# austin-hoover/ment-flow

Measured on NVIDIA B200. Metric: particles/sec/GPU for flow sample+log_prob+project+KDE (6D, 100 proj), higher is better.
Workload: dtype f32

## Files before the change

include/mentflow_b200.h:

```cpp
#ifndef MENTFLOW_B200_H
#define MENTFLOW_B200_H

#include <stdint.h>

#ifdef __cplusplus
extern "C" {
#endif

#define MFB_ABI_VERSION 2

#define MFB_E_BADARG (-1)
#define MFB_E_UNSUPPORTED (-2)
#define MFB_E_WORKSPACE (-3)

#define MFB_FLAG_NO_TENSOR_CORES 1

int mfb_abi_version(void);
const char* mfb_error_string(int code);
int mfb_sm_count(void);

#define MFB_GEOM_STRIDE 8

int64_t mfb_kde1d_workspace_bytes(int64_t n, int d, int k, int b);
int mfb_project_kde1d_fwd(const float* x, int64_t n, int d, const float* proj, const float* geom,
// ... 133 lines not shown
                          int nb_meas2, int meas_axis2, int n_int_axes, const int32_t* int_shape_host,
                          const float* int_first_host, const float* int_step_host, const float* minv,
                          const float* proj, const float* coords, const float* tables, int k, int b,
                          const float* proj2, const float* cx2, const float* cy2, const float* tables2, int k2,
                          int bx, int by, float prior_neg_half_inv_s2, float prior_log_norm, float* pred,
                          void* stream);
int64_t mfb_cdf_workspace_bytes(int64_t g);
int mfb_cdf_build(const float* rho, int64_t g, double pad, double* cdf, void* workspace,
                  int64_t workspace_bytes, void* stream);
int mfb_cdf_sample(const double* cdf, int64_t g, const void* workspace, int d,
                   const int32_t* shape_host, const float* first_edge_host, const float* cell_host,
                   int jitter, uint64_t seed, uint64_t offset, int64_t size, float* out, void* stream);
int mfb_gs_update(float* table, const float* meas, const float* pred, int n, float lr, float thresh,
                  void* stream);

int64_t mfb_randn_offset_increment(int64_t numel);
int mfb_randn_philox(float* out, int64_t numel, uint64_t seed, uint64_t offset, void* stream);
int mfb_randn_philox_state(float* out, int64_t numel, uint64_t* state, int advance, void* stream);

int mfb_selftest_umma(const float* a, const float* b, int n, float* d, int* err, void* stream);
int mfb_selftest_umma_ts(const float* a, const float* b, int n, float* d, int* err, void* stream);
int mfb_selftest_umma_sw32(const float* a, const float* b, int n, int mode, int kstep, float* d, int* err,
                           void* stream);

#ifdef __cplusplus
}
#endif
#endif
```

mentflow_b200/_lib.py:

```python
import ctypes
import os
from ctypes import c_char_p, c_double, c_float, c_int, c_int64, c_uint64, c_void_p

PKG_DIR = os.path.dirname(os.path.abspath(__file__))
LIB_PATH = os.environ.get("MENTFLOW_B200_LIB") or os.path.join(PKG_DIR, "libmentflow_b200.so")

P = c_void_p

SIGNATURES = {
    "mfb_abi_version": (c_int, []),
    "mfb_error_string": (c_char_p, [c_int]),
    "mfb_sm_count": (c_int, []),
    "mfb_kde1d_workspace_bytes": (c_int64, [c_int64, c_int, c_int, c_int]),
    "mfb_project_kde1d_fwd": (c_int, [P, c_int64, c_int, P, P, c_int, c_int, c_float, P, P, c_int64, P]),
    "mfb_kde1d_normalize": (c_int, [P, c_double, P, c_int, c_int, P, P]),
    "mfb_kde1d_normalize_bwd": (c_int, [P, c_double, P, c_int, c_int, P, P, P]),
    "mfb_project_kde1d_loss_fwd": (c_int, [P, c_int64, c_int, P, P, c_int, c_int, c_float, c_double, P, c_float, P, P, P,
                                           P, c_int64, P]),
    "mfb_kde1d_finish": (c_int, [P, c_double, P, c_int, c_int, P, c_float, P, P, P]),
    "mfb_kde1d_p2p_block_floats": (c_int64, [c_int, c_int, c_int]),
    "mfb_kde1d_finish_p2p": (c_int, [P, c_int, c_int, P, P, P, c_int, c_double, P, c_int, c_int, P, c_float, P, P, P, P, P]),
    "mfb_project_kde1d_loss_fwd_p2p": (c_int, [P, c_int64, c_int, P, P, c_int, c_int, c_float, c_double, P, c_float, P,
                                               c_int, c_int, P, P, c_int, P, P, P, P, P, c_int64, P]),
    "mfb_kde1d_finish_bwd": (c_int, [P, c_double, P, c_int, c_int, P, c_float, P, P, P, P]),
# ... 23 lines not shown
                                  c_int64, c_int, P]),
    "mfb_nsf_layer_bwd_img": (c_int, [P, P, P, c_int64, c_int, c_int, c_int, c_int, P, P, P, c_int, P, P, P, c_int, P,
                                      c_int64, c_int, P]),
    "mfb_ment_prob": (c_int, [P, c_int64, c_int, P, P, P, c_int, c_int, c_float, c_float, P, P]),
    "mfb_ment_prob_grid": (c_int, [c_int, P, P, P, P, P, P, c_int, c_int, c_float, c_float, P, P]),
    "mfb_ment_integrate": (c_int, [c_int, P, c_int, c_int, c_int, P, P, P, P, P, P, P, c_int, c_int, c_float,
                                   c_float, P, P]),
    "mfb_ment_prob_nd": (c_int, [P, c_int64, c_int, P, P, P, c_int, c_int, P, P, P, P, c_int, c_int, c_int, c_float,
                                 c_float, P, P]),
    "mfb_ment_prob_grid_nd": (c_int, [c_int, P, P, P, P, P, P, c_int, c_int, P, P, P, P, c_int, c_int, c_int, c_float,
                                      c_float, P, P]),
    "mfb_ment_integrate_nd": (c_int, [c_int, P, c_int, c_int, P, c_int, c_int, c_int, P, P, P, P, P, P, P, c_int, c_int,
                                      P, P, P, P, c_int, c_int, c_int, c_float, c_float, P, P]),
    "mfb_randn_offset_increment": (c_int64, [c_int64]),
    "mfb_randn_philox": (c_int, [P, c_int64, c_uint64, c_uint64, P]),
    "mfb_randn_philox_state": (c_int, [P, c_int64, P, c_int, P]),
    "mfb_cdf_workspace_bytes": (c_int64, [c_int64]),
    "mfb_cdf_build": (c_int, [P, c_int64, c_double, P, P, c_int64, P]),
    "mfb_cdf_sample": (c_int, [P, c_int64, P, c_int, P, P, P, c_int, c_uint64, c_uint64, c_int64, P, P]),
    "mfb_gs_update": (c_int, [P, P, P, c_int, c_float, c_float, P]),
    "mfb_selftest_umma": (c_int, [P, P, c_int, P, P, P]),
    "mfb_selftest_umma_ts": (c_int, [P, P, c_int, P, P, P]),
    "mfb_selftest_umma_sw32": (c_int, [P, P, c_int, c_int, c_int, P, P, P]),
    "mfb_nsf_pack_params": (c_int, [P, P, P, P, P, P, P, P, P, c_int, c_int, c_int, c_int, c_int, P, P, P]),
    "mfb_nsf_unpack_grads": (c_int, [P, P, P, P, c_int, c_int, c_int, c_int, c_int, P, P, P, P, P, P, P]),
    "mfb_moments_workspace_bytes": (c_int64, [c_int64, c_int]),
    "mfb_moments": (c_int, [P, P, c_int64, c_int, c_int, P, P, c_int64, P]),
    "mfb_f64_split": (c_int, [P, c_int, P, P]),
    "mfb_f64_join": (c_int, [P, c_int, P, P]),
    "mfb_mc_entropy": (c_int, [P, c_double, c_double, c_double, P, P]),
    "mfb_loss_tail": (c_int, [P, c_int, P, c_float, P, P]),
}

_lib = None


class LibraryMissing(RuntimeError):
    pass


def load():
    global _lib
    if _lib is not None:
        return _lib
    if not os.path.exists(LIB_PATH):
        raise LibraryMissing(
# ... 19 lines not shown
```

mentflow_b200/csrc/nsf_spline_regs.cuh:

```cuda
#pragma once
#include <math.h>

#include "nsf_common.cuh"

#define MFB_HD __host__ __device__ __forceinline__

namespace mfb {
namespace tc {

constexpr int kCT = 24;
constexpr int kConstRows = 7;
constexpr int kConstFloats = kConstRows * kCT + kPP;

MFB_HD float sp_exp2(float x) {
#ifdef __CUDA_ARCH__
  float y;
  asm("ex2.approx.ftz.f32 %0, %1;" : "=f"(y) : "f"(x));
  return y;
#else
  return exp2f(x);
#endif
}
MFB_HD float sp_rcp(float x) {
#ifdef __CUDA_ARCH__
// ... 64 lines not shown
  const float d2 = fmaf(fabsf(t2), c, 1.0f), d3 = fmaf(fabsf(t3), c, 1.0f);
  float p01, p23, x0, x1, x2, x3;
  mul2(d0, d2, d1, d3, p01, p23);
  const float r = sp_rcp(p01 * p23);
  const float r01 = r * p23, r23 = r * p01;
  mul2(t0, t1, r01 * d1, r01 * d0, x0, x1);
  mul2(t2, t3, r23 * d3, r23 * d2, x2, x3);
  e0 = sp_exp2(x0);
  e1 = sp_exp2(x1);
  e2 = sp_exp2(x2);
  e3 = sp_exp2(x3);
}

MFB_HD void two_sum(float a, float b, float& s, float& err) {
  s = sp_add(a, b);
  const float bb = sp_add(s, -a);
  err = sp_add(sp_add(a, -sp_add(s, -bb)), sp_add(b, -bb));
}

#ifndef MFB_SPLINE_COMP
#define MFB_SPLINE_COMP 1
#endif

template <int NB>
MFB_HD float rq_spline_regs(const float (&a)[64], float v, float& jac) {
  static_assert(NB % 4 == 0 && NB >= 8, "bins are searched in groups of four");
  constexpr int G = NB / 4;
  constexpr float cW = kClipW / kLog2e, cD = kClipD / kLog2e;
  float e[NB], pre[G + 1], plo[G + 1];
#pragma unroll
  for (int j = 0; j < NB; j += 4) {
    clip_exp2_quad(a[j], a[j + 1], a[j + 2], a[j + 3], cW, e[j], e[j + 1], e[j + 2], e[j + 3]);
  }
  pre[0] = 0.f;
  plo[0] = 0.f;
#pragma unroll
  for (int g = 0; g < G; ++g) {
    float s01, s23;
    add2(e[4 * g], e[4 * g + 2], e[4 * g + 1], e[4 * g + 3], s01, s23);
    const float gs = s01 + s23;
    if (MFB_SPLINE_COMP >= 1 && g > 0) {
      float err;
      two_sum(pre[g], gs, pre[g + 1], err);
      plo[g + 1] = plo[g] + err;
    } else {
      pre[g + 1] = pre[g] + gs;
      plo[g + 1] = 0.f;
    }
  }
  const float sum = pre[G], half = 0.5f * sum;
  const float u = v * (0.5f / kBound);
  const float target = fmaf(u, sum, half);
  bool pg[G - 1];
#pragma unroll
  for (int g = 0; g < G - 1; ++g) pg[g] = pre[g + 1] < target;
  float q0 = e[0], q1 = e[1], q2 = e[2], q3 = e[3], xg = 0.f, xgl = 0.f;
#pragma unroll
  for (int g = 1; g < G; ++g) {
    q0 = pg[g - 1] ? e[4 * g] : q0;
    q1 = pg[g - 1] ? e[4 * g + 1] : q1;
    q2 = pg[g - 1] ? e[4 * g + 2] : q2;
    q3 = pg[g - 1] ? e[4 * g + 3] : q3;
    xg = pg[g - 1] ? pre[g] : xg;
    if (MFB_SPLINE_COMP >= 1) xgl = pg[g - 1] ? plo[g] : xgl;
  }
  float cen = half - xg;
  if (MFB_SPLINE_COMP >= 1) cen += fmaf(0.5f, plo[G], -xgl);
  const float rem = fmaf(u, sum, cen);
  const float i1 = q0 + q1, i2 = i1 + q2;
  const bool r0 = q0 < rem, r1 = i1 < rem, r2 = i2 < rem;
  const float numer = rem - (r2 ? i2 : (r1 ? i1 : (r0 ? q0 : 0.f)));
  const float ek = r2 ? q3 : (r1 ? q2 : (r0 ? q1 : q0));
  float run = 0.f, runl = 0.f, yg = 0.f, ygl = 0.f, h0s = 0.f, h1s = 0.f, h2s = 0.f, h3s = 0.f;
#pragma unroll
  for (int g = 0; g < G; ++g) {
    float h0, h1, h2, h3;
    clip_exp2_quad(a[NB + 4 * g], a[NB + 4 * g + 1], a[NB + 4 * g + 2], a[NB + 4 * g + 3], cW, h0, h1, h2, h3);
    const bool take = g == 0 ? true : pg[g > 0 ? g - 1 : 0];
    h0s = take ? h0 : h0s;
    h1s = take ? h1 : h1s;
    h2s = take ? h2 : h2s;
    h3s = take ? h3 : h3s;
    yg = take ? run : yg;
    float s01, s23;
    add2(h0, h2, h1, h3, s01, s23);
    const float gs = s01 + s23;
    if (MFB_SPLINE_COMP >= 2 && g > 0) {
      ygl = take ? runl : ygl;
      float err;
      two_sum(run, gs, run, err);
      runl += err;
    } else {
      run += gs;
    }
  }
  const float sumh = run;
  const float j1h = h0s + h1s, j2h = j1h + h2s;
  float ycen = (yg - 0.5f * sumh) + (r2 ? j2h : (r1 ? j1h : (r0 ? h0s : 0.f)));
  if (MFB_SPLINE_COMP >= 2) ycen += fmaf(-0.5f, runl, ygl);
  const float hk = r2 ? h3s : (r1 ? h2s : (r0 ? h1s : h0s));
  float um = 0.f, u0 = 0.f, u1 = 0.f, u2 = 0.f, u3 = 0.f, prev = 0.f;
#pragma unroll
  for (int g = 0; g < G; ++g) {
    const float t0 = a[2 * NB + 4 * g], t1 = a[2 * NB + 4 * g + 1], t2 = a[2 * NB + 4 * g + 2];
    const float t3 = (4 * g + 3 < NB - 1) ? a[2 * NB + 4 * g + 3] : 0.f;
    const bool take = g == 0 ? true : pg[g > 0 ? g - 1 : 0];
    um = take ? prev : um;
    u0 = take ? t0 : u0;
    u1 = take ? t1 : u1;
    u2 = take ? t2 : u2;
    u3 = take ? t3 : u3;
    prev = t3;
  }
  const float tl = r2 ? u2 : (r1 ? u1 : (r0 ? u0 : um));
  const float tr = r2 ? u3 : (r1 ? u2 : (r0 ? u1 : u0));
  float d0, d1;
  clip_exp2_pair(tl, tr, cD, d0, d1);
  const float r_e = rcp_nr(ek), r_sh = rcp_nr(sumh);
  float t = numer * r_e;
  t = fminf(fmaxf(t, 0.0f), 1.0f);
  const float hn = hk * r_sh;
  const float s = hn * sum * r_e;
  const float omt = 1.0f - t, tomt = t * omt;
  const float den = fmaf(d0 + d1 - 2.0f * s, tomt, s);
  const float r_den = rcp_nr(den);
  const float y0 = 2.0f * kBound * (ycen * r_sh);
  const float y = fmaf(2.0f * kBound * hn * (s * t * t + d0 * tomt), r_den, y0);
  const float j1 = s * s * (2.0f * s * tomt + d0 * omt * omt + d1 * t * t) * r_den * r_den;
  const bool inside = (v > -kBound) && (v <= kBound);
  jac *= inside ? j1 : 1.0f;
  return inside ? y : v;
}

MFB_HD void clip_exp2_quad_bwd(float& t0, float& t1, float& t2, float& t3, float c, float& e0,
                                                   float& e1, float& e2, float& e3) {
  const float d0 = fmaf(fabsf(t0), c, 1.0f), d1 = fmaf(fabsf(t1), c, 1.0f);
  const float d2 = fmaf(fabsf(t2), c, 1.0f), d3 = fmaf(fabsf(t3), c, 1.0f);
  const float p01 = d0 * d1, p23 = d2 * d3;
  const float r = sp_rcp(p01 * p23);
  const float r01 = r * p23, r23 = r * p01;
  const float i0 = r01 * d1, i1 = r01 * d0, i2 = r23 * d3, i3 = r23 * d2;
  e0 = sp_exp2(t0 * i0);
  e1 = sp_exp2(t1 * i1);
  e2 = sp_exp2(t2 * i2);
  e3 = sp_exp2(t3 * i3);
  t0 = i0; t1 = i1; t2 = i2; t3 = i3;
}

struct KnotGrad {
  float left, right;
  int bin;
};
template <int NB>
MFB_HD float rq_spline_regs_bwd(float (&a)[64], float v, float gy, float gl, KnotGrad* kg = nullptr) {
// ... 242 lines not shown
```

mentflow_b200/csrc/nsf_tc.cu:

```cuda
#include "nsf_spline_regs.cuh"
#include "nsf_tc_common.cuh"

namespace mfb {
namespace tc {


struct Meta {
  int slot_feature[kMaxDim];
  int slot_ksteps[kMaxDim];
  int hid_n0[4];
  int const_feature;
  int nslots;
  int perm[kH];
};

struct BwdIO {
  const float* gy;
  const float* glogq;
  float* acts;
  float* gphi;
  uint32_t* masks;
  float* gvd;
  float* gmax;
  int* gmaxes;
// ... 194 lines not shown
  asm("cvt.rz.relu.f16x2.f32 %0, %1, %2;" : "=r"(hi) : "f"(x1), "f"(x0));
  const __half2 h = *reinterpret_cast<const __half2*>(&hi);
  const float2 hf = __half22float2(h);
  float r0, r1;
  add2(x0, x1, -hf.x, -hf.y, r0, r1);
  asm("cvt.rn.relu.f16x2.f32 %0, %1, %2;" : "=r"(lo) : "f"(r1), "f"(r0));
}

__device__ __forceinline__ void store_hidden(const float (&acc)[64], unsigned char* a_hi, unsigned char* a_lo, int row) {
#pragma unroll
  for (int c = 0; c < 8; ++c) {
    uint32_t hi[4], lo[4];
#pragma unroll
    for (int e = 0; e < 4; ++e) split_relu_pair(acc[8 * c + 2 * e], acc[8 * c + 2 * e + 1], hi[e], lo[e]);
    const uint32_t off = umma::sw128_offset(row, c);
    *reinterpret_cast<uint4*>(a_hi + off) = make_uint4(hi[0], hi[1], hi[2], hi[3]);
    *reinterpret_cast<uint4*>(a_lo + off) = make_uint4(lo[0], lo[1], lo[2], lo[3]);
  }
}

#ifndef MFB_TC_TS
#define MFB_TC_TS 1
#endif
__device__ __forceinline__ void store_hidden_ts(const float (&acc)[64], uint32_t tmem_a_hi, unsigned char* a_lo, int row) {
#pragma unroll
  for (int c2 = 0; c2 < 4; ++c2) {
    uint32_t hi[8];
#pragma unroll
    for (int h = 0; h < 2; ++h) {
      const int c = 2 * c2 + h;
      uint32_t lo[4];
#pragma unroll
      for (int e = 0; e < 4; ++e) split_relu_pair(acc[8 * c + 2 * e], acc[8 * c + 2 * e + 1], hi[4 * h + e], lo[e]);
      *reinterpret_cast<uint4*>(a_lo + umma::sw128_offset(row, c)) = make_uint4(lo[0], lo[1], lo[2], lo[3]);
    }
    umma::tmem_st8(tmem_a_hi + 8 * c2, hi);
  }
  umma::tmem_wait_st();
}

__device__ __forceinline__ void mirror_rows(const unsigned char* a_hi, unsigned char* g_img, int warp_in_wg) {
  __syncwarp();
  if ((threadIdx.x & 31) == 0) {
    const uint32_t off = (uint32_t)warp_in_wg * 4096u;
    asm volatile("cp.async.bulk.global.shared::cta.bulk_group [%0], [%1], 4096;" ::"l"(g_img + off), "r"(smem_u32(a_hi + off)) : "memory");
    asm volatile("cp.async.bulk.global.shared::cta.bulk_group [%0], [%1], 4096;" ::"l"(g_img + kABytes / 2 + off),
                 "r"(smem_u32(a_hi + kABytes / 2 + off))
                 : "memory");
    asm volatile("cp.async.bulk.commit_group;" ::: "memory");
  }
}
__device__ __forceinline__ void mirror_wait() {
  if ((threadIdx.x & 31) == 0) asm volatile("cp.async.bulk.wait_group.read 0;" ::: "memory");
  __syncwarp();
}

__device__ __forceinline__ void mma_slot(uint32_t tmem_d, uint64_t a_hi, uint64_t a_lo, uint64_t b_hi, uint64_t b_lo,
                                         int nk, uint32_t idesc) {
  for (int ks = 0; ks < nk; ++ks) mma_cross(tmem_d, a_hi, a_lo, b_hi, b_lo, ks, idesc, ks > 0);
  for (int ks = 0; ks < nk; ++ks) mma_main(tmem_d, a_hi, b_hi, ks, idesc);
}
// ... 189 lines not shown
    umma::fence_after_sync();
    TRACE(2);
  };
  auto start_tile = [&](const float* vv, uint64_t* landed, uint32_t parity) {
    mbar_wait_bounded(landed, parity);
    if constexpr (kBwd) mirror_wait();
    __align__(16) __half row[16];
#pragma unroll
    for (int e = 0; e < 16; ++e) row[e] = __float2half_rn(0.f);
#pragma unroll
    for (int i = 0; i < D; ++i) umma::split_f16(vv[i], row[i], row[D + i]);
    row[2 * D] = __float2half_rn(1.0f);
    row[2 * D + 1] = __float2half_rn(1.0f);
    *reinterpret_cast<uint4*>(a_hi + umma::sw128_offset(t, 0)) = reinterpret_cast<const uint4*>(row)[0];
    *reinterpret_cast<uint4*>(a_hi + umma::sw128_offset(t, 1)) = reinterpret_cast<const uint4*>(row)[1];
    fence_proxy_async();
    request_arrive(req_chain);
    TRACE(3);
  };
  int64_t next_p = 0;
  bool next_valid = false;
  auto hidden_step = [&](int l) {
    wait_buf(kHB);
    float acc[64];
    tmem_ld64(col0 + (uint32_t)(kHB * 64) + lane_sel, acc);
    if constexpr (kBwd) mirror_wait();
    if constexpr (kTS) store_hidden_ts(acc, ta_hi + lane_sel, a_lo, t);
    else store_hidden(acc, a_hi, a_lo, t);
    fence_proxy_async();
    umma::fence_before_sync();
    request_arrive(req_chain);
    if constexpr (kBwd) {
      mirror_rows(a_hi, reinterpret_cast<unsigned char*>(bio.acts) + ((size_t)(next_p >> 7) * L + l) * kABytes, t >> 5);
      if (next_valid) {
        uint32_t m0 = 0, m1 = 0;
#pragma unroll
        for (int c = 0; c < 64; ++c) {
          if (c < 32) m0 |= (acc[c] > 0.f ? 1u : 0u) << c;
          else m1 |= (acc[c] > 0.f ? 1u : 0u) << (c - 32);
        }
        uint32_t* mk = bio.masks + ((size_t)(next_p >> 7) * (L * 2) + l * 2) * 128 + t;
        mk[0] = m0;
        mk[128] = m1;
      }
    }
    TRACE(4 + l);
  };

  float* stage0 = stage_all + ((size_t)(wg * 2) * 128 + t) * D;
  float* stage1 = stage0 + 128 * D;
  uint64_t* sbar = sbars + 2 * wg;
// ... 10 lines not shown
    if (bulk) tma_load_1d(dst, src, bulk, &sbar[buf]);
  };

  int64_t tile = first_tile_of(wg);
  bool cur = false;
  bool has_next = tile < ntiles;
  float* sc = stage0;
  float* sn = stage1;
  int nbuf = 1;
  uint32_t sph0 = 0, sph1 = 0;
  float jac_carry = 1.0f, ss_carry = 0.f;
  if (t == 0) prefetch(tile, nbuf);
  tile -= tstride;
  while (cur || has_next) {
    const int64_t p = tile * 128 + t;
    const bool valid = cur && p < n;
    if (cur) has_next = tile + tstride < ntiles;
    next_p = (tile + tstride) * 128 + t;
    next_valid = has_next && next_p < n;
    float jac = jac_carry;
    float ss = ss_carry;
    float lq_in = 0.f;
    if (!kBwd && cur && valid && logq_out && !first_layer) lq_in = logq_in[p];
    float gyr[D], glq = 0.f, amax = 0.f;
    if constexpr (kBwd) {
#pragma unroll
      for (int i = 0; i < D; ++i) gyr[i] = valid ? bio.gy[p * D + i] : 0.f;
      glq = (valid && bio.glogq) ? bio.glogq[p] : 0.f;
    }
    auto feature_bwd = [&](float (&acc)[64], int f) {
      const float vf = sc[f];
      float gyf = gyr[0];
#pragma unroll
      for (int i = 1; i < D; ++i) gyf = (f == i) ? gyr[i] : gyf;
      KnotGrad kg;
      float gvf = rq_spline_regs_bwd<NB>(acc, vf, gyf, -glq, &kg);
      if (first_layer) gvf -= glq * vf;
      sc[f] = gvf;
      if (valid) {
        float* gp = bio.gphi + ((size_t)tile * (D * kGRows) + f * kGRows) * 128 + t;
#pragma unroll
        for (int j = 0; j < 2 * NB; ++j) {
          gp[j * 128] = acc[j];
          amax = fmaxf(amax, fabsf(acc[j]));
        }
        gp[(2 * NB) * 128] = kg.left;
        gp[(2 * NB + 1) * 128] = kg.right;
        gp[(2 * NB + 2) * 128] = (float)kg.bin;
        amax = fmaxf(amax, fmaxf(fabsf(kg.left), fabsf(kg.right)));
      }
    };
#pragma unroll 1
    for (int s = kBwd ? -1 : 0; s < S; ++s) {
      const int b = s & 1;
      float acc[64];
      if (kBwd && s < 0) {
        if (cur) {
          const float4* cb = reinterpret_cast<const float4*>(ctab + kConstRows * kCT);
#pragma unroll
          for (int i = 0; i < 16; ++i) {
            const float4 q4 = cb[i];
            acc[4 * i] = q4.x; acc[4 * i + 1] = q4.y; acc[4 * i + 2] = q4.z; acc[4 * i + 3] = q4.w;
          }
        }
      } else if (cur) {
        if (!(S >= 2 && s == S - 1)) wait_buf(b);
        tmem_ld64(col0 + (uint32_t)(b * 64) + lane_sel, acc);
        umma::fence_before_sync();
        if (s + 2 < S) request_arrive(req_chain + 1 + b);
        if (s == 0 && t == 0 && has_next) prefetch(tile + tstride, nbuf);
        TRACE(10 + s);
      }
      if (s == kFork) {
        if (cur && S >= 2) wait_buf((S - 1) & 1);
        if (has_next) {
          if (nbuf == 0) {
            start_tile(sn, &sbar[0], sph0);
            sph0 ^= 1;
          } else {
            start_tile(sn, &sbar[1], sph1);
            sph1 ^= 1;
          }
        }
      }
      if (cur) {
        const int f = (kBwd && s < 0) ? meta.const_feature : meta.slot_feature[s < 0 ? 0 : s];
        if constexpr (kBwd) {
          feature_bwd(acc, f);
        } else {
          const float vf = sc[f];
          ss = fmaf(vf, vf, ss);
          sc[f] = rq_spline_regs<NB>(acc, vf, jac);
        }
        TRACE(20 + s);
      }
      if (has_next) {
        if (s == kFork) hidden_step(0);
        if (S >= 2 && s == S - 1) hidden_step(1);
      }
    }
    if (S == 1 && has_next) hidden_step(1);
    if constexpr (kBwd) {
      if (valid) {
#pragma unroll
        for (int i = 0; i < D; ++i) bio.gvd[p * D + i] = sc[i];
        bio.gmax[p] = amax;
      }
      if (cur) {
        float wm = valid ? amax : 0.f;
#pragma unroll
        for (int o = 16; o > 0; o >>= 1) wm = fmaxf(wm, __shfl_xor_sync(0xffffffffu, wm, o));
        if ((t & 31) == 0) atomicMax(bio.gmaxes, __float_as_int(wm));
      }
      if (has_next) hidden_step(2);
    } else {
      if (valid) {
#pragma unroll
// ... 471 lines not shown
```

mentflow_b200/csrc/nsf_tc_common.cuh:

```cuda
#pragma once
#include "nsf_common.cuh"
#include "umma.cuh"

namespace mfb {
namespace tc {

constexpr int kWG = 3;
constexpr int kThreads = (kWG + 1) * 128;
constexpr int kRegsCompute = 160, kRegsIssuer = 32;
constexpr int kTileBytes = 8192;
constexpr int kABytes = 32768;
constexpr int kGRowsOf(int nb) { return 2 * nb + 4; }
constexpr int kGRows = kGRowsOf(20);

#ifndef MFB_TC_DEAL_BY_WG
#define MFB_TC_DEAL_BY_WG 1
#endif
__device__ __forceinline__ int64_t first_tile_of(int wg) {
#if MFB_TC_DEAL_BY_WG
  return (int64_t)wg * gridDim.x + blockIdx.x;
#else
  return (int64_t)blockIdx.x * kWG + wg;
#endif
}
// ... 49 lines not shown
__device__ __forceinline__ void tmem_ld64(uint32_t taddr, float (&v)[64]) {
  uint32_t r[64];
  asm volatile(
      "tcgen05.ld.sync.aligned.32x32b.x64.b32 "
      "{%0, %1, %2, %3, %4, %5, %6, %7, %8, %9, %10, %11, %12, %13, %14, %15, "
      "%16, %17, %18, %19, %20, %21, %22, %23, %24, %25, %26, %27, %28, %29, %30, %31, "
      "%32, %33, %34, %35, %36, %37, %38, %39, %40, %41, %42, %43, %44, %45, %46, %47, "
      "%48, %49, %50, %51, %52, %53, %54, %55, %56, %57, %58, %59, %60, %61, %62, %63}, [%64];"
      : "=r"(r[0]), "=r"(r[1]), "=r"(r[2]), "=r"(r[3]), "=r"(r[4]), "=r"(r[5]), "=r"(r[6]), "=r"(r[7]), "=r"(r[8]),
        "=r"(r[9]), "=r"(r[10]), "=r"(r[11]), "=r"(r[12]), "=r"(r[13]), "=r"(r[14]), "=r"(r[15]), "=r"(r[16]),
        "=r"(r[17]), "=r"(r[18]), "=r"(r[19]), "=r"(r[20]), "=r"(r[21]), "=r"(r[22]), "=r"(r[23]), "=r"(r[24]),
        "=r"(r[25]), "=r"(r[26]), "=r"(r[27]), "=r"(r[28]), "=r"(r[29]), "=r"(r[30]), "=r"(r[31]), "=r"(r[32]),
        "=r"(r[33]), "=r"(r[34]), "=r"(r[35]), "=r"(r[36]), "=r"(r[37]), "=r"(r[38]), "=r"(r[39]), "=r"(r[40]),
        "=r"(r[41]), "=r"(r[42]), "=r"(r[43]), "=r"(r[44]), "=r"(r[45]), "=r"(r[46]), "=r"(r[47]), "=r"(r[48]),
        "=r"(r[49]), "=r"(r[50]), "=r"(r[51]), "=r"(r[52]), "=r"(r[53]), "=r"(r[54]), "=r"(r[55]), "=r"(r[56]),
        "=r"(r[57]), "=r"(r[58]), "=r"(r[59]), "=r"(r[60]), "=r"(r[61]), "=r"(r[62]), "=r"(r[63])
      : "r"(taddr)
      : "memory");
  asm volatile("tcgen05.wait::ld.sync.aligned;" ::: "memory");
#pragma unroll
  for (int i = 0; i < 64; ++i) v[i] = __uint_as_float(r[i]);
}

__device__ __forceinline__ void mma_cross(uint32_t tmem_d, uint64_t a_hi, uint64_t a_lo, uint64_t b_hi, uint64_t b_lo,
                                          int kstep, uint32_t idesc, uint32_t accumulate) {
  umma::mma_f16_ss(tmem_d, umma::desc_advance_k(a_hi, kstep), umma::desc_advance_k(b_lo, kstep), idesc, accumulate);
  umma::mma_f16_ss(tmem_d, umma::desc_advance_k(a_lo, kstep), umma::desc_advance_k(b_hi, kstep), idesc, 1);
}
__device__ __forceinline__ void mma_main(uint32_t tmem_d, uint64_t a_hi, uint64_t b_hi, int kstep, uint32_t idesc) {
  umma::mma_f16_ss(tmem_d, umma::desc_advance_k(a_hi, kstep), umma::desc_advance_k(b_hi, kstep), idesc, 1);
}
__device__ __forceinline__ void store_split8(unsigned char* hi_tile, unsigned char* lo_tile, int row, int chunk,
                                             const float (&x)[8]) {
  __align__(16) __half hi[8], lo[8];
#pragma unroll
  for (int e = 0; e < 8; ++e) umma::split_f16(x[e], hi[e], lo[e]);
  const uint32_t off = umma::sw128_offset(row, chunk);
  *reinterpret_cast<uint4*>(hi_tile + off) = *reinterpret_cast<const uint4*>(hi);
  *reinterpret_cast<uint4*>(lo_tile + off) = *reinterpret_cast<const uint4*>(lo);
}
static void hidden_classes(int d, int* cls, int* perm) {
  for (int h = 0; h < kH; ++h) cls[h] = 1 + h % (d - 1);
  int p = 0;
  for (int c = 1; c <= d - 1; ++c)
    for (int h = 0; h < kH; ++h)
      if (cls[h] == c) perm[p++] = h;
// ... 5 lines not shown
```

mentflow_b200/csrc/umma.cuh:

```cuda
#pragma once
#include <cuda_fp16.h>

#include "common.cuh"

namespace mfb {
namespace umma {

__device__ __forceinline__ uint32_t sw128_offset(int r, int c) {
  return (uint32_t)((r >> 3) * 1024 + (r & 7) * 128 + ((c ^ (r & 7)) << 4));
}

__device__ __forceinline__ uint64_t make_desc_sw128(uint32_t smem_addr) {
  uint64_t d = (uint64_t)((smem_addr & 0x3FFFFu) >> 4);
  d |= (uint64_t)1 << 16;
  d |= (uint64_t)(1024 >> 4) << 32;
  d |= (uint64_t)1 << 46;
  d |= (uint64_t)2 << 61;
  return d;
}
__device__ __forceinline__ uint64_t desc_advance_k(uint64_t desc, int kstep) { return desc + (uint64_t)(kstep * 2); }

__device__ __forceinline__ uint32_t sw32_offset(int r, int c) {
  return (uint32_t)(r * 32 + ((c ^ ((r >> 2) & 1)) << 4));
}
// ... 50 lines not shown
}
__device__ __forceinline__ void tmem_st4(uint32_t taddr, const uint32_t (&r)[4]) {
  asm volatile("tcgen05.st.sync.aligned.32x32b.x4.b32 [%0], {%1, %2, %3, %4};" ::"r"(taddr), "r"(r[0]), "r"(r[1]), "r"(r[2]),
               "r"(r[3])
               : "memory");
}
__device__ __forceinline__ void tmem_wait_st() { asm volatile("tcgen05.wait::st.sync.aligned;" ::: "memory"); }
__device__ __forceinline__ void commit(uint64_t* bar) {
  asm volatile("tcgen05.commit.cta_group::1.mbarrier::arrive::one.shared::cluster.b64 [%0];" ::"r"(smem_u32(bar))
               : "memory");
}
__device__ __forceinline__ void fence_before_sync() { asm volatile("tcgen05.fence::before_thread_sync;" ::: "memory"); }
__device__ __forceinline__ void fence_after_sync() { asm volatile("tcgen05.fence::after_thread_sync;" ::: "memory"); }

__device__ __forceinline__ void tmem_alloc(uint32_t* dst, uint32_t cols) {
  asm volatile("tcgen05.alloc.cta_group::1.sync.aligned.shared::cta.b32 [%0], %1;" ::"r"(smem_u32(dst)), "r"(cols)
               : "memory");
  asm volatile("tcgen05.relinquish_alloc_permit.cta_group::1.sync.aligned;" ::: "memory");
}
__device__ __forceinline__ void tmem_dealloc(uint32_t addr, uint32_t cols) {
  asm volatile("tcgen05.dealloc.cta_group::1.sync.aligned.b32 %0, %1;" ::"r"(addr), "r"(cols) : "memory");
}

__device__ __forceinline__ void tmem_ld32(uint32_t taddr, float (&v)[32]) {
  uint32_t r[32];
  asm volatile(
      "tcgen05.ld.sync.aligned.32x32b.x32.b32 "
      "{%0, %1, %2, %3, %4, %5, %6, %7, %8, %9, %10, %11, %12, %13, %14, %15, "
      "%16, %17, %18, %19, %20, %21, %22, %23, %24, %25, %26, %27, %28, %29, %30, %31}, [%32];"
      : "=r"(r[0]), "=r"(r[1]), "=r"(r[2]), "=r"(r[3]), "=r"(r[4]), "=r"(r[5]), "=r"(r[6]), "=r"(r[7]), "=r"(r[8]),
        "=r"(r[9]), "=r"(r[10]), "=r"(r[11]), "=r"(r[12]), "=r"(r[13]), "=r"(r[14]), "=r"(r[15]), "=r"(r[16]),
        "=r"(r[17]), "=r"(r[18]), "=r"(r[19]), "=r"(r[20]), "=r"(r[21]), "=r"(r[22]), "=r"(r[23]), "=r"(r[24]),
        "=r"(r[25]), "=r"(r[26]), "=r"(r[27]), "=r"(r[28]), "=r"(r[29]), "=r"(r[30]), "=r"(r[31])
      : "r"(taddr)
      : "memory");
  asm volatile("tcgen05.wait::ld.sync.aligned;" ::: "memory");
#pragma unroll
  for (int i = 0; i < 32; ++i) v[i] = __uint_as_float(r[i]);
}

__device__ __forceinline__ void split_f16(float x, __half& hi, __half& lo) {
  hi = __float2half_rn(x);
  lo = __float2half_rn(x - __half2float(hi));
}

}
// ... 2 lines not shown
```

mentflow_b200/csrc/umma_selftest.cu:

```cuda
#include "umma.cuh"

namespace mfb {

constexpr int kSelfWaitLimit = 1 << 22;

__global__ void __launch_bounds__(128, 1)
umma_selftest_kernel(const float* __restrict__ A, const float* __restrict__ B, int N, float* __restrict__ D,
                     int* __restrict__ err) {
  extern __shared__ __align__(1024) unsigned char smem[];
  unsigned char* a_hi = smem;
  unsigned char* a_lo = smem + 16384;
  unsigned char* b_hi = smem + 32768;
  unsigned char* b_lo = b_hi + (size_t)N * 128;
  __shared__ uint64_t bar;
  __shared__ uint32_t tmem_base;
  const int tid = threadIdx.x;

  if (tid == 0) {
    mbar_init(&bar, 1);
    fence_mbar_init();
  }
  if (tid < 32) umma::tmem_alloc(&tmem_base, 256);
  for (int r = tid; r < 128 + N; r += 128) {
    const bool isA = r < 128;
// ... 177 lines not shown
      umma::mma_f16_ts(tbase, tbase + 160 + 8 * k, umma::desc_advance_k(db_hi, k), idesc, 1);
    }
    umma::commit(&bar);
  }
  int spins = 0;
  while (!mbar_try_wait(&bar, 0)) {
    if (++spins > kSelfWaitLimit) {
      if (tid == 0) *err = 1;
      break;
    }
  }
  umma::fence_after_sync();
  for (int c0 = 0; c0 < N; c0 += 32) {
    float v[32];
    umma::tmem_ld32(tbase + ((uint32_t)(warp * 32) << 16) + (uint32_t)c0, v);
#pragma unroll
    for (int i = 0; i < 32; ++i) D[(size_t)tid * N + c0 + i] = v[i];
  }
  umma::fence_before_sync();
  __syncthreads();
  if (tid < 32) umma::tmem_dealloc(tbase, 256);
}

}

extern "C" int mfb_selftest_umma_ts(const float* a, const float* b, int n, float* d, int* err, void* stream) {
  MFB_CHECK_ARG(a && b && d && err && (n == 64 || n == 96 || n == 128));
  const size_t smem = (size_t)n * 256 + 1024;
  MFB_CUDA(cudaFuncSetAttribute(mfb::umma_selftest_ts_kernel, cudaFuncAttributeMaxDynamicSharedMemorySize, (int)smem));
  mfb::umma_selftest_ts_kernel<<<1, 128, smem, (cudaStream_t)stream>>>(a, b, n, d, err);
  return mfb::launch_status();
}

extern "C" int mfb_selftest_umma_sw32(const float* a, const float* b, int n, int mode, int kstep, float* d, int* err,
                                      void* stream) {
  MFB_CHECK_ARG(a && b && d && err && (n == 64 || n == 128) && (mode == 0 || mode == 1) && kstep >= 0 && kstep < 4);
  const size_t smem = 4096 + 16384 + (size_t)n * 32 + 1024;
  MFB_CUDA(cudaFuncSetAttribute(mfb::umma_selftest_sw32_kernel, cudaFuncAttributeMaxDynamicSharedMemorySize, (int)smem));
  mfb::umma_selftest_sw32_kernel<<<1, 128, smem, (cudaStream_t)stream>>>(a, b, n, mode, kstep, d, err);
  return mfb::launch_status();
}

extern "C" int mfb_selftest_umma(const float* a, const float* b, int n, float* d, int* err, void* stream) {
  MFB_CHECK_ARG(a && b && d && err && (n == 64 || n == 128 || n == 256));
  const size_t smem = 32768 + (size_t)n * 256 + 1024;
  MFB_CUDA(cudaFuncSetAttribute(mfb::umma_selftest_kernel, cudaFuncAttributeMaxDynamicSharedMemorySize, (int)smem));
// ... 4 lines not shown
```

Before: 847.0 million.

## Load TMEM accumulators in pieces for spline and hidden-layer stores in forward

In the forward NSF tensor-core kernel, the spline evaluator now pulls its parameters from tensor memory in two stages: widths first, then heights and derivatives, through a loader callback. The buffer-release signalling is moved into the second load. The hidden-layer store also processes the accumulator in two 32-column halves instead of one 64-float array. These changes are meant to lower peak register pressure and let the buffer be released while spline math continues, at the cost of more tcgen05.ld/wait round trips. Separately, it adds cluster-pair (cta_group::2) UMMA helpers and a selftest kernel, which the main path does not use.

After: 912.1 million, median of 6. +7.7%, better.

```diff
diff --git a/include/mentflow_b200.h b/include/mentflow_b200.h
--- a/include/mentflow_b200.h
+++ b/include/mentflow_b200.h
@@ -179,6 +179,7 @@
 int mfb_selftest_umma_ts(const float* a, const float* b, int n, float* d, int* err, void* stream);
 int mfb_selftest_umma_sw32(const float* a, const float* b, int n, int mode, int kstep, float* d, int* err,
                            void* stream);
+int mfb_selftest_umma_pair(const float* a, const float* b, int mode, float* d, int* err, void* stream);
 
 #ifdef __cplusplus
 }
diff --git a/mentflow_b200/_lib.py b/mentflow_b200/_lib.py
--- a/mentflow_b200/_lib.py
+++ b/mentflow_b200/_lib.py
@@ -69,6 +69,7 @@
     "mfb_selftest_umma": (c_int, [P, P, c_int, P, P, P]),
     "mfb_selftest_umma_ts": (c_int, [P, P, c_int, P, P, P]),
     "mfb_selftest_umma_sw32": (c_int, [P, P, c_int, c_int, c_int, P, P, P]),
+    "mfb_selftest_umma_pair": (c_int, [P, P, c_int, P, P, P]),
     "mfb_nsf_pack_params": (c_int, [P, P, P, P, P, P, P, P, P, c_int, c_int, c_int, c_int, c_int, P, P, P]),
     "mfb_nsf_unpack_grads": (c_int, [P, P, P, P, c_int, c_int, c_int, c_int, c_int, P, P, P, P, P, P, P]),
     "mfb_moments_workspace_bytes": (c_int64, [c_int64, c_int]),
diff --git a/mentflow_b200/csrc/nsf_spline_regs.cuh b/mentflow_b200/csrc/nsf_spline_regs.cuh
--- a/mentflow_b200/csrc/nsf_spline_regs.cuh
+++ b/mentflow_b200/csrc/nsf_spline_regs.cuh
@@ -110,15 +110,19 @@
 #define MFB_SPLINE_COMP 1
 #endif
 
-template <int NB>
-MFB_HD float rq_spline_regs(const float (&a)[64], float v, float& jac) {
+template <int NB, class Load>
+MFB_HD float rq_spline_regs_ld(Load&& load, float v, float& jac) {
   static_assert(NB % 4 == 0 && NB >= 8, "bins are searched in groups of four");
   constexpr int G = NB / 4;
   constexpr float cW = kClipW / kLog2e, cD = kClipD / kLog2e;
   float e[NB], pre[G + 1], plo[G + 1];
-#pragma unroll
-  for (int j = 0; j < NB; j += 4) {
-    clip_exp2_quad(a[j], a[j + 1], a[j + 2], a[j + 3], cW, e[j], e[j + 1], e[j + 2], e[j + 3]);
+  {
+    float aw[NB];
+    load(0, aw);
+#pragma unroll
+    for (int j = 0; j < NB; j += 4) {
+      clip_exp2_quad(aw[j], aw[j + 1], aw[j + 2], aw[j + 3], cW, e[j], e[j + 1], e[j + 2], e[j + 3]);
+    }
   }
   pre[0] = 0.f;
   plo[0] = 0.f;
@@ -159,11 +163,13 @@
   const bool r0 = q0 < rem, r1 = i1 < rem, r2 = i2 < rem;
   const float numer = rem - (r2 ? i2 : (r1 ? i1 : (r0 ? q0 : 0.f)));
   const float ek = r2 ? q3 : (r1 ? q2 : (r0 ? q1 : q0));
+  float a[2 * NB];
+  load(NB, a);
   float run = 0.f, runl = 0.f, yg = 0.f, ygl = 0.f, h0s = 0.f, h1s = 0.f, h2s = 0.f, h3s = 0.f;
 #pragma unroll
   for (int g = 0; g < G; ++g) {
     float h0, h1, h2, h3;
-    clip_exp2_quad(a[NB + 4 * g], a[NB + 4 * g + 1], a[NB + 4 * g + 2], a[NB + 4 * g + 3], cW, h0, h1, h2, h3);
+    clip_exp2_quad(a[4 * g], a[4 * g + 1], a[4 * g + 2], a[4 * g + 3], cW, h0, h1, h2, h3);
     const bool take = g == 0 ? true : pg[g > 0 ? g - 1 : 0];
     h0s = take ? h0 : h0s;
     h1s = take ? h1 : h1s;
@@ -190,8 +196,8 @@
   float um = 0.f, u0 = 0.f, u1 = 0.f, u2 = 0.f, u3 = 0.f, prev = 0.f;
 #pragma unroll
   for (int g = 0; g < G; ++g) {
-    const float t0 = a[2 * NB + 4 * g], t1 = a[2 * NB + 4 * g + 1], t2 = a[2 * NB + 4 * g + 2];
-    const float t3 = (4 * g + 3 < NB - 1) ? a[2 * NB + 4 * g + 3] : 0.f;
+    const float t0 = a[NB + 4 * g], t1 = a[NB + 4 * g + 1], t2 = a[NB + 4 * g + 2];
+    const float t3 = (4 * g + 3 < NB - 1) ? a[NB + 4 * g + 3] : 0.f;
     const bool take = g == 0 ? true : pg[g > 0 ? g - 1 : 0];
     um = take ? prev : um;
     u0 = take ? t0 : u0;
@@ -218,6 +224,14 @@
   const bool inside = (v > -kBound) && (v <= kBound);
   jac *= inside ? j1 : 1.0f;
   return inside ? y : v;
+}
+template <int NB>
+MFB_HD float rq_spline_regs(const float (&a)[64], float v, float& jac) {
+  return rq_spline_regs_ld<NB>(
+      [&](int col, auto& dst) {
+        for (int j = 0; j < (int)(sizeof(dst) / sizeof(dst[0])); ++j) dst[j] = a[col + j];
+      },
+      v, jac);
 }
 
 MFB_HD void clip_exp2_quad_bwd(float& t0, float& t1, float& t2, float& t3, float c, float& e0,
diff --git a/mentflow_b200/csrc/nsf_tc.cu b/mentflow_b200/csrc/nsf_tc.cu
--- a/mentflow_b200/csrc/nsf_tc.cu
+++ b/mentflow_b200/csrc/nsf_tc.cu
@@ -240,21 +240,24 @@
 #ifndef MFB_TC_TS
 #define MFB_TC_TS 1
 #endif
-__device__ __forceinline__ void store_hidden_ts(const float (&acc)[64], uint32_t tmem_a_hi, unsigned char* a_lo, int row) {
-#pragma unroll
-  for (int c2 = 0; c2 < 4; ++c2) {
+template <bool kTS>
+__device__ __forceinline__ void store_hidden_piece(const float (&acc)[32], int piece, uint32_t tmem_a_hi,
+                                                   unsigned char* a_hi, unsigned char* a_lo, int row) {
+#pragma unroll
+  for (int c2 = 0; c2 < 2; ++c2) {
     uint32_t hi[8];
 #pragma unroll
     for (int h = 0; h < 2; ++h) {
-      const int c = 2 * c2 + h;
+      const int cl = 2 * c2 + h, c = 4 * piece + cl;
       uint32_t lo[4];
 #pragma unroll
-      for (int e = 0; e < 4; ++e) split_relu_pair(acc[8 * c + 2 * e], acc[8 * c + 2 * e + 1], hi[4 * h + e], lo[e]);
+      for (int e = 0; e < 4; ++e) split_relu_pair(acc[8 * cl + 2 * e], acc[8 * cl + 2 * e + 1], hi[4 * h + e], lo[e]);
       *reinterpret_cast<uint4*>(a_lo + umma::sw128_offset(row, c)) = make_uint4(lo[0], lo[1], lo[2], lo[3]);
-    }
-    umma::tmem_st8(tmem_a_hi + 8 * c2, hi);
-  }
-  umma::tmem_wait_st();
+      if constexpr (!kTS)
+        *reinterpret_cast<uint4*>(a_hi + umma::sw128_offset(row, c)) = make_uint4(hi[4 * h], hi[4 * h + 1], hi[4 * h + 2], hi[4 * h + 3]);
+    }
+    if constexpr (kTS) umma::tmem_st8(tmem_a_hi + 8 * (2 * piece + c2), hi);
+  }
 }
 
 __device__ __forceinline__ void mirror_rows(const unsigned char* a_hi, unsigned char* g_img, int warp_in_wg) {
@@ -490,11 +493,20 @@
   bool next_valid = false;
   auto hidden_step = [&](int l) {
     wait_buf(kHB);
-    float acc[64];
-    tmem_ld64(col0 + (uint32_t)(kHB * 64) + lane_sel, acc);
-    if constexpr (kBwd) mirror_wait();
-    if constexpr (kTS) store_hidden_ts(acc, ta_hi + lane_sel, a_lo, t);
-    else store_hidden(acc, a_hi, a_lo, t);
+    float acc[kBwd ? 64 : 1];
+    if constexpr (kBwd) {
+      tmem_ld64(col0 + (uint32_t)(kHB * 64) + lane_sel, acc);
+      mirror_wait();
+      store_hidden(acc, a_hi, a_lo, t);
+    } else {
+#pragma unroll
+      for (int piece = 0; piece < 2; ++piece) {
+        float part[32];
+        tmem_ld_cols(col0 + (uint32_t)(kHB * 64 + 32 * piece) + lane_sel, part);
+        store_hidden_piece<kTS>(part, piece, ta_hi + lane_sel, a_hi, a_lo, t);
+      }
+      if constexpr (kTS) umma::tmem_wait_st();
+    }
     fence_proxy_async();
     umma::fence_before_sync();
     request_arrive(req_chain);
@@ -551,7 +563,7 @@
     float ss = ss_carry;
     float lq_in = 0.f;
     if (!kBwd && cur && valid && logq_out && !first_layer) lq_in = logq_in[p];
-    float gyr[D], glq = 0.f, amax = 0.f;
+    float gyr[D] = {}, glq = 0.f, amax = 0.f;
     if constexpr (kBwd) {
 #pragma unroll
       for (int i = 0; i < D; ++i) gyr[i] = valid ? bio.gy[p * D + i] : 0.f;
@@ -582,25 +594,7 @@
 #pragma unroll 1
     for (int s = kBwd ? -1 : 0; s < S; ++s) {
       const int b = s & 1;
-      float acc[64];
-      if (kBwd && s < 0) {
-        if (cur) {
-          const float4* cb = reinterpret_cast<const float4*>(ctab + kConstRows * kCT);
-#pragma unroll
-          for (int i = 0; i < 16; ++i) {
-            const float4 q4 = cb[i];
-            acc[4 * i] = q4.x; acc[4 * i + 1] = q4.y; acc[4 * i + 2] = q4.z; acc[4 * i + 3] = q4.w;
-          }
-        }
-      } else if (cur) {
-        if (!(S >= 2 && s == S - 1)) wait_buf(b);
-        tmem_ld64(col0 + (uint32_t)(b * 64) + lane_sel, acc);
-        umma::fence_before_sync();
-        if (s + 2 < S) request_arrive(req_chain + 1 + b);
-        if (s == 0 && t == 0 && has_next) prefetch(tile + tstride, nbuf);
-        TRACE(10 + s);
-      }
-      if (s == kFork) {
+      auto fork = [&]() {
         if (cur && S >= 2) wait_buf((S - 1) & 1);
         if (has_next) {
           if (nbuf == 0) {
@@ -611,17 +605,52 @@
             sph1 ^= 1;
           }
         }
-      }
-      if (cur) {
-        const int f = (kBwd && s < 0) ? meta.const_feature : meta.slot_feature[s < 0 ? 0 : s];
-        if constexpr (kBwd) {
-          feature_bwd(acc, f);
-        } else {
-          const float vf = sc[f];
-          ss = fmaf(vf, vf, ss);
-          sc[f] = rq_spline_regs<NB>(acc, vf, jac);
-        }
+      };
+      auto slot_ready = [&]() {
+        if (!(S >= 2 && s == S - 1)) wait_buf(b);
+        if (s == 0 && t == 0 && has_next) prefetch(tile + tstride, nbuf);
+      };
+      if constexpr (kBwd) {
+        float acc[64];
+        if (s < 0) {
+          if (cur) {
+            const float4* cb = reinterpret_cast<const float4*>(ctab + kConstRows * kCT);
+#pragma unroll
+            for (int i = 0; i < 16; ++i) {
+              const float4 q4 = cb[i];
+              acc[4 * i] = q4.x; acc[4 * i + 1] = q4.y; acc[4 * i + 2] = q4.z; acc[4 * i + 3] = q4.w;
+            }
+          }
+        } else if (cur) {
+          slot_ready();
+          tmem_ld64(col0 + (uint32_t)(b * 64) + lane_sel, acc);
+          umma::fence_before_sync();
+          if (s + 2 < S) request_arrive(req_chain + 1 + b);
+          TRACE(10 + s);
+        }
+        if (s == kFork) fork();
+        if (cur) {
+          feature_bwd(acc, s < 0 ? meta.const_feature : meta.slot_feature[s < 0 ? 0 : s]);
+          TRACE(20 + s);
+        }
+      } else if (cur) {
+        slot_ready();
+        const int f = meta.slot_feature[s];
+        const float vf = sc[f];
+        ss = fmaf(vf, vf, ss);
+        sc[f] = rq_spline_regs_ld<NB>(
+            [&](int col, auto& dst) {
+              tmem_ld_cols(col0 + (uint32_t)(b * 64 + col) + lane_sel, dst);
+              if (col == 0) return;
+              umma::fence_before_sync();
+              if (s + 2 < S) request_arrive(req_chain + 1 + b);
+              TRACE(10 + s);
+              if (s == kFork) fork();
+            },
+            vf, jac);
         TRACE(20 + s);
+      } else if (s == kFork) {
+        fork();
       }
       if (has_next) {
         if (s == kFork) hidden_step(0);
diff --git a/mentflow_b200/csrc/nsf_tc_common.cuh b/mentflow_b200/csrc/nsf_tc_common.cuh
--- a/mentflow_b200/csrc/nsf_tc_common.cuh
+++ b/mentflow_b200/csrc/nsf_tc_common.cuh
@@ -95,6 +95,55 @@
   for (int i = 0; i < 64; ++i) v[i] = __uint_as_float(r[i]);
 }
 
+template <int W>
+__device__ __forceinline__ void tmem_ld_issue(uint32_t taddr, uint32_t* r) {
+  static_assert(W == 4 || W == 8 || W == 16 || W == 32, "tcgen05.ld widths used here");
+  if constexpr (W == 4) {
+    asm volatile("tcgen05.ld.sync.aligned.32x32b.x4.b32 {%0, %1, %2, %3}, [%4];"
+                 : "=r"(r[0]), "=r"(r[1]), "=r"(r[2]), "=r"(r[3])
+                 : "r"(taddr)
+                 : "memory");
+  } else if constexpr (W == 8) {
+    asm volatile("tcgen05.ld.sync.aligned.32x32b.x8.b32 {%0, %1, %2, %3, %4, %5, %6, %7}, [%8];"
+                 : "=r"(r[0]), "=r"(r[1]), "=r"(r[2]), "=r"(r[3]), "=r"(r[4]), "=r"(r[5]), "=r"(r[6]), "=r"(r[7])
+                 : "r"(taddr)
+                 : "memory");
+  } else if constexpr (W == 16) {
+    asm volatile(
+        "tcgen05.ld.sync.aligned.32x32b.x16.b32 "
+        "{%0, %1, %2, %3, %4, %5, %6, %7, %8, %9, %10, %11, %12, %13, %14, %15}, [%16];"
+        : "=r"(r[0]), "=r"(r[1]), "=r"(r[2]), "=r"(r[3]), "=r"(r[4]), "=r"(r[5]), "=r"(r[6]), "=r"(r[7]), "=r"(r[8]),
+          "=r"(r[9]), "=r"(r[10]), "=r"(r[11]), "=r"(r[12]), "=r"(r[13]), "=r"(r[14]), "=r"(r[15])
+        : "r"(taddr)
+        : "memory");
+  } else {
+    asm volatile(
+        "tcgen05.ld.sync.aligned.32x32b.x32.b32 "
+        "{%0, %1, %2, %3, %4, %5, %6, %7, %8, %9, %10, %11, %12, %13, %14, %15, "
+        "%16, %17, %18, %19, %20, %21, %22, %23, %24, %25, %26, %27, %28, %29, %30, %31}, [%32];"
+        : "=r"(r[0]), "=r"(r[1]), "=r"(r[2]), "=r"(r[3]), "=r"(r[4]), "=r"(r[5]), "=r"(r[6]), "=r"(r[7]), "=r"(r[8]),
+          "=r"(r[9]), "=r"(r[10]), "=r"(r[11]), "=r"(r[12]), "=r"(r[13]), "=r"(r[14]), "=r"(r[15]), "=r"(r[16]),
+          "=r"(r[17]), "=r"(r[18]), "=r"(r[19]), "=r"(r[20]), "=r"(r[21]), "=r"(r[22]), "=r"(r[23]), "=r"(r[24]),
+          "=r"(r[25]), "=r"(r[26]), "=r"(r[27]), "=r"(r[28]), "=r"(r[29]), "=r"(r[30]), "=r"(r[31])
+        : "r"(taddr)
+        : "memory");
+  }
+}
+template <int N>
+__device__ __forceinline__ void tmem_ld_cols(uint32_t taddr, float (&v)[N]) {
+  static_assert(N % 4 == 0 && N <= 64, "pieces of 4 to 64 columns");
+  uint32_t r[N];
+  int c = 0;
+#pragma unroll
+  for (; c + 32 <= N; c += 32) tmem_ld_issue<32>(taddr + c, r + c);
+  if constexpr ((N & 16) != 0) { tmem_ld_issue<16>(taddr + c, r + c); c += 16; }
+  if constexpr ((N & 8) != 0) { tmem_ld_issue<8>(taddr + c, r + c); c += 8; }
+  if constexpr ((N & 4) != 0) { tmem_ld_issue<4>(taddr + c, r + c); }
+  asm volatile("tcgen05.wait::ld.sync.aligned;" ::: "memory");
+#pragma unroll
+  for (int i = 0; i < N; ++i) v[i] = __uint_as_float(r[i]);
+}
+
 __device__ __forceinline__ void mma_cross(uint32_t tmem_d, uint64_t a_hi, uint64_t a_lo, uint64_t b_hi, uint64_t b_lo,
                                           int kstep, uint32_t idesc, uint32_t accumulate) {
   umma::mma_f16_ss(tmem_d, umma::desc_advance_k(a_hi, kstep), umma::desc_advance_k(b_lo, kstep), idesc, accumulate);
diff --git a/mentflow_b200/csrc/umma.cuh b/mentflow_b200/csrc/umma.cuh
--- a/mentflow_b200/csrc/umma.cuh
+++ b/mentflow_b200/csrc/umma.cuh
@@ -96,6 +96,62 @@
   asm volatile("tcgen05.dealloc.cta_group::1.sync.aligned.b32 %0, %1;" ::"r"(addr), "r"(cols) : "memory");
 }
 
+__device__ __forceinline__ uint32_t cluster_rank() {
+  uint32_t r;
+  asm volatile("mov.u32 %0, %%cluster_ctarank;" : "=r"(r));
+  return r;
+}
+__device__ __forceinline__ void cluster_sync() {
+  asm volatile("barrier.cluster.arrive.release.aligned;\nbarrier.cluster.wait.acquire.aligned;" ::: "memory");
+}
+__device__ __forceinline__ uint32_t cluster_addr(const void* p, uint32_t rank) {
+  uint32_t a;
+  asm volatile("mapa.shared::cluster.u32 %0, %1, %2;" : "=r"(a) : "r"(smem_u32(p)), "r"(rank));
+  return a;
+}
+__device__ __forceinline__ void mbar_arrive_cluster(uint32_t cluster_bar) {
+  asm volatile("mbarrier.arrive.release.cluster.shared::cluster.b64 _, [%0];" ::"r"(cluster_bar) : "memory");
+}
+__device__ __forceinline__ bool mbar_try_wait_cluster(uint64_t* bar, uint32_t parity) {
+  uint32_t ok;
+  asm volatile(
+      "{\n"
+      ".reg .pred p;\n"
+      "mbarrier.try_wait.parity.acquire.cluster.shared::cta.b64 p, [%1], %2;\n"
+      "selp.u32 %0, 1, 0, p;\n"
+      "}\n"
+      : "=r"(ok)
+      : "r"(smem_u32(bar)), "r"(parity)
+      : "memory");
+  return ok != 0;
+}
+__device__ __forceinline__ void mma_f16_ss_pair(uint32_t tmem_d, uint64_t adesc, uint64_t bdesc, uint32_t idesc,
+                                                uint32_t accumulate) {
+  asm volatile(
+      "{\n"
+      ".reg .pred p;\n"
+      "setp.ne.b32 p, %4, 0;\n"
+      "tcgen05.mma.cta_group::2.kind::f16 [%0], %1, %2, %3, p;\n"
+      "}\n" ::"r"(tmem_d),
+      "l"(adesc), "l"(bdesc), "r"(idesc), "r"(accumulate)
+      : "memory");
+}
+__device__ __forceinline__ void commit_pair(uint64_t* bar) {
+  asm volatile(
+      "tcgen05.commit.cta_group::2.mbarrier::arrive::one.shared::cluster.multicast::cluster.b64 [%0], %1;" ::"r"(
+          smem_u32(bar)),
+      "h"((uint16_t)3)
+      : "memory");
+}
+__device__ __forceinline__ void tmem_alloc_pair(uint32_t* dst, uint32_t cols) {
+  asm volatile("tcgen05.alloc.cta_group::2.sync.aligned.shared::cta.b32 [%0], %1;" ::"r"(smem_u32(dst)), "r"(cols)
+               : "memory");
+  asm volatile("tcgen05.relinquish_alloc_permit.cta_group::2.sync.aligned;" ::: "memory");
+}
+__device__ __forceinline__ void tmem_dealloc_pair(uint32_t addr, uint32_t cols) {
+  asm volatile("tcgen05.dealloc.cta_group::2.sync.aligned.b32 %0, %1;" ::"r"(addr), "r"(cols) : "memory");
+}
+
 __device__ __forceinline__ void tmem_ld32(uint32_t taddr, float (&v)[32]) {
   uint32_t r[32];
   asm volatile(
diff --git a/mentflow_b200/csrc/umma_selftest.cu b/mentflow_b200/csrc/umma_selftest.cu
--- a/mentflow_b200/csrc/umma_selftest.cu
+++ b/mentflow_b200/csrc/umma_selftest.cu
@@ -223,6 +223,100 @@
   if (tid < 32) umma::tmem_dealloc(tbase, 256);
 }
 
+__global__ void __launch_bounds__(128, 1)
+umma_selftest_pair_kernel(const float* __restrict__ A, const float* __restrict__ B, int mode, float* __restrict__ D,
+                          int* __restrict__ err) {
+  extern __shared__ unsigned char smem_raw[];
+  unsigned char* smem = smem_raw + ((1024u - (smem_u32(smem_raw) & 1023u)) & 1023u);
+  unsigned char* a_t = smem;
+  unsigned char* b_t = smem + 16384;
+  uint64_t* bars = reinterpret_cast<uint64_t*>(smem + 16384 + 4096);
+  uint32_t* tmem_slot = reinterpret_cast<uint32_t*>(bars + 2);
+  const int tid = threadIdx.x, K = mode == 0 ? 16 : 64;
+  const uint32_t rank = umma::cluster_rank();
+  if (tid == 0) {
+    mbar_init(&bars[0], 1);
+    mbar_init(&bars[1], 2);
+    fence_mbar_init();
+  }
+  if (tid < 32) umma::tmem_alloc_pair(tmem_slot, 64);
+  for (int r = tid; r < 128 + 32; r += 128) {
+    const bool isA = r < 128;
+    const int row = isA ? r : r - 128;
+    const float* src = isA ? A + (size_t)(128 * rank + row) * K : B + (size_t)(32 * rank + row) * K;
+    for (int c = 0; c < K / 8; ++c) {
+      __align__(16) __half h[8];
+#pragma unroll
+      for (int e = 0; e < 8; ++e) h[e] = __float2half_rn(src[c * 8 + e]);
+      const uint32_t off = mode == 0 ? umma::sw32_offset(row, c) : umma::sw128_offset(row, c);
+      *reinterpret_cast<uint4*>((isA ? a_t : b_t) + off) = *reinterpret_cast<const uint4*>(h);
+    }
+  }
+  fence_proxy_async();
+  umma::fence_before_sync();
+  umma::cluster_sync();
+  umma::fence_after_sync();
+  const uint32_t tbase = *tmem_slot;
+  if (tid == 0) umma::mbar_arrive_cluster(umma::cluster_addr(&bars[1], 0));
+  if (rank == 0 && tid == 0) {
+    int spins = 0;
+    while (!umma::mbar_try_wait_cluster(&bars[1], 0)) {
+      if (++spins > kSelfWaitLimit) {
+        *err = 2;
+        break;
+      }
+    }
+    umma::fence_after_sync();
+    const uint32_t idesc = umma::make_idesc_f16(256, 64);
+    if (mode == 0) {
+      umma::mma_f16_ss_pair(tbase, umma::make_desc_sw32(smem_u32(a_t)), umma::make_desc_sw32(smem_u32(b_t)), idesc, 0);
+    } else {
+      const uint64_t da = umma::make_desc_sw128(smem_u32(a_t)), db = umma::make_desc_sw128(smem_u32(b_t));
+      for (int k = 0; k < 4; ++k)
+        umma::mma_f16_ss_pair(tbase, umma::desc_advance_k(da, k), umma::desc_advance_k(db, k), idesc, k > 0);
+    }
+    umma::commit_pair(&bars[0]);
+  }
+  int spins = 0;
+  while (!mbar_try_wait(&bars[0], 0)) {
+    if (++spins > kSelfWaitLimit) {
+      if (tid == 0) *err = 1;
+      break;
+    }
+  }
+  umma::fence_after_sync();
+  const int warp = tid >> 5;
+  for (int c0 = 0; c0 < 64; c0 += 32) {
+    float v[32];
+    umma::tmem_ld32(tbase + ((uint32_t)(warp * 32) << 16) + (uint32_t)c0, v);
+#pragma unroll
+    for (int i = 0; i < 32; ++i) D[(size_t)(128 * rank + tid) * 64 + c0 + i] = v[i];
+  }
+  umma::fence_before_sync();
+  umma::cluster_sync();
+  if (tid < 32) umma::tmem_dealloc_pair(tbase, 64);
+}
+
+}
+
+extern "C" int mfb_selftest_umma_pair(const float* a, const float* b, int mode, float* d, int* err, void* stream) {
+  MFB_CHECK_ARG(a && b && d && err && (mode == 0 || mode == 1));
+  const size_t smem = 16384 + 4096 + 64 + 1024;
+  MFB_CUDA(cudaFuncSetAttribute(mfb::umma_selftest_pair_kernel, cudaFuncAttributeMaxDynamicSharedMemorySize, (int)smem));
+  cudaLaunchConfig_t cfg = {};
+  cfg.gridDim = dim3(2);
+  cfg.blockDim = dim3(128);
+  cfg.dynamicSmemBytes = smem;
+  cfg.stream = (cudaStream_t)stream;
+  cudaLaunchAttribute attr[1];
+  attr[0].id = cudaLaunchAttributeClusterDimension;
+  attr[0].val.clusterDim.x = 2;
+  attr[0].val.clusterDim.y = 1;
+  attr[0].val.clusterDim.z = 1;
+  cfg.attrs = attr;
+  cfg.numAttrs = 1;
+  MFB_CUDA(cudaLaunchKernelEx(&cfg, mfb::umma_selftest_pair_kernel, a, b, mode, d, err));
+  return mfb::launch_status();
 }
 
 extern "C" int mfb_selftest_umma_ts(const float* a, const float* b, int n, float* d, int* err, void* stream) {
```
